# chungongyu/siga

Hardware: AMD Instinct MI355X
Metric: reads/sec overlapped (ASQG bit-exact) (higher is better)
Workload: dtype u64

## Files before the change

siga_amd/csrc/sigax_kernels.hip:

```cpp
#include <hip/hip_runtime.h>

#include <cstdlib>

#include "sigax_kernels.h"

typedef unsigned long long u64;
typedef unsigned int u32;

#ifndef SIGAX_NT
#define SIGAX_NT 7
#endif

struct Cnt4 {
  u64 a, c, g, t;
};

template <bool WIDE> struct PosOf { typedef u32 type; };
template <> struct PosOf<true> { typedef u64 type; };
template <typename P> struct Cnt4P {
  P a, c, g, t;
};

template <bool WIDE> struct Cand;
template <> struct __attribute__((aligned(32))) Cand<false> {
// ... 604 lines not shown
      }
      return true;
    }
    slot = slot + 1 == nslots ? 0 : slot + 1;
  }
}

__device__ __forceinline__ void store_block(sigax_block* dst, u64 c0lo, u64 c0hi, u64 c1lo, u64 c1hi, u64 r0lo, u64 r0hi,
                                            u64 r1lo, u64 r1hi, u32 len, u32 af) {
  ulonglong2* d = reinterpret_cast<ulonglong2*>(dst);
  d[0] = make_ulonglong2(c0lo, c0hi);
  d[1] = make_ulonglong2(c1lo, c1hi);
  d[2] = make_ulonglong2(r0lo, r0hi);
  d[3] = make_ulonglong2(r1lo, r1hi);
  d[4] = make_ulonglong2((u64)len | ((u64)af << 32), 0ull);
}

template <bool WIDE>
__global__ __launch_bounds__(256) void k_build2_a(FmStrand s, u32* gran2, u32* cnt, u64 ng2) {
  const FmRef F = fm_ref(s, 0);
  const u32 lane = threadIdx.x & 63u;
  const u64 wave = ((u64)blockIdx.x * 256 + threadIdx.x) >> 6, nw = (u64)gridDim.x * 4;
  for (u64 g = wave; g < ng2; g += nw) {
    const u64 p = g * 64 + lane;
    u32 c1 = 0, c2 = 0;
    if (p < s.n) {
      c1 = fm_char(F, p);
      if (c1 >= 1 && c1 <= 4) {
        const Cnt4 k = fm_rank<WIDE>(F, p);
        const u64 rk = c1 == 1 ? k.a : c1 == 2 ? k.c : c1 == 3 ? k.g : k.t;
        c2 = fm_char(F, s.C[c1] + rk);
      } else {
        c1 = c1 > 4 ? 0 : c1;
      }
    }
    const u64 y1 = __ballot((c1 & 1u) != 0), z1 = __ballot((c1 & 2u) != 0), w1 = __ballot((c1 & 4u) != 0);
    const u64 y2 = __ballot((c2 & 1u) != 0), z2 = __ballot((c2 & 2u) != 0), w2 = __ballot((c2 & 4u) != 0);
    u32 mine = 0;
    for (u32 b = 1; b <= 4; ++b) {
      const u32 v = (u32)__popcll(__ballot(c1 == b));
      if (lane == b - 1) mine = v;
    }
    for (u32 c = 1; c <= 4; ++c)
      for (u32 x = 1; x <= 4; ++x) {
        const u32 v = (u32)__popcll(__ballot(c1 == c && c2 == x));
        if (lane == 4 + (c - 1) * 4 + (x - 1)) mine = v;
      }
    if (lane < 20) cnt[(u64)lane * ng2 + g] = mine;
    if (lane == 0) {
      u32* q = gran2 + g * SIGAX_GRAN2_WORDS + 20;
      q[0] = (u32)y1; q[1] = (u32)(y1 >> 32); q[2] = (u32)z1; q[3] = (u32)(z1 >> 32); q[4] = (u32)w1; q[5] = (u32)(w1 >> 32);
      q[6] = (u32)y2; q[7] = (u32)(y2 >> 32); q[8] = (u32)z2; q[9] = (u32)(z2 >> 32); q[10] = (u32)w2; q[11] = (u32)(w2 >> 32);
    }
  }
}
__global__ __launch_bounds__(256) void k_build2_b(const u64* offs, u32* gran2, u32 col, u64 ng2, u64* super2) {
  const u64 g = (u64)blockIdx.x * 256 + threadIdx.x;
  if (g >= ng2) return;
  u64 base = 0;
  if (super2) {
    const u32 sh = SIGAX_SUPER_SHIFT - 6;
    const u64 first = (g >> sh) << sh;
    base = offs[first];
    if (g == first) super2[(g >> sh) * 20 + col] = base;
  }
  gran2[g * SIGAX_GRAN2_WORDS + col] = (u32)(offs[g] - base);
}

#ifndef SIGAX_FIND_POLICY
#define SIGAX_FIND_POLICY ""
#endif
struct Gran2 {
  v4u s, pc, p5, p6, p7;
};
__device__ __forceinline__ void find_step2_loads(const void* base, u32 offa, u32 offa_c, u32 offb, u32 offb_c, Gran2& a, Gran2& b) {
  asm volatile(
      "global_load_dwordx4 %0, %10, %14" SIGAX_FIND_POLICY "\n\t"
      "global_load_dwordx4 %5, %12, %14" SIGAX_FIND_POLICY "\n\t"
      "global_load_dwordx4 %1, %11, %14" SIGAX_FIND_POLICY "\n\t"
      "global_load_dwordx4 %2, %10, %14 offset:80" SIGAX_FIND_POLICY "\n\t"
      "global_load_dwordx4 %3, %10, %14 offset:96" SIGAX_FIND_POLICY "\n\t"
      "global_load_dwordx4 %4, %10, %14 offset:112" SIGAX_FIND_POLICY "\n\t"
      "global_load_dwordx4 %6, %13, %14" SIGAX_FIND_POLICY "\n\t"
      "global_load_dwordx4 %7, %12, %14 offset:80" SIGAX_FIND_POLICY "\n\t"
      "global_load_dwordx4 %8, %12, %14 offset:96" SIGAX_FIND_POLICY "\n\t"
      "global_load_dwordx4 %9, %12, %14 offset:112" SIGAX_FIND_POLICY "\n\t"
      "s_waitcnt vmcnt(0)"
      : "=&v"(a.s), "=&v"(a.pc), "=&v"(a.p5), "=&v"(a.p6), "=&v"(a.p7), "=&v"(b.s), "=&v"(b.pc), "=&v"(b.p5), "=&v"(b.p6),
        "=&v"(b.p7)
      : "v"(offa), "v"(offa_c), "v"(offb), "v"(offb_c), "s"(base)
      : "memory");
}
__device__ __forceinline__ void find_step2_loads_masked(const void* base, u32 offa, u32 offa_c, u32 offb, u32 offb_c, u64 two, Gran2& a,
                                                        Gran2& b) {
  u64 saved;
  asm volatile(
      "global_load_dwordx4 %0, %11, %15" SIGAX_FIND_POLICY "\n\t"
      "global_load_dwordx4 %1, %12, %15" SIGAX_FIND_POLICY "\n\t"
      "global_load_dwordx4 %2, %11, %15 offset:80" SIGAX_FIND_POLICY "\n\t"
      "global_load_dwordx4 %3, %11, %15 offset:96" SIGAX_FIND_POLICY "\n\t"
      "global_load_dwordx4 %4, %11, %15 offset:112" SIGAX_FIND_POLICY "\n\t"
      "s_and_saveexec_b64 %10, %16\n\t"
      "global_load_dwordx4 %5, %13, %15" SIGAX_FIND_POLICY "\n\t"
      "global_load_dwordx4 %6, %14, %15" SIGAX_FIND_POLICY "\n\t"
      "global_load_dwordx4 %7, %13, %15 offset:80" SIGAX_FIND_POLICY "\n\t"
      "global_load_dwordx4 %8, %13, %15 offset:96" SIGAX_FIND_POLICY "\n\t"
      "global_load_dwordx4 %9, %13, %15 offset:112" SIGAX_FIND_POLICY "\n\t"
      "s_mov_b64 exec, %10\n\t"
      "s_waitcnt vmcnt(0)"
      : "=&v"(a.s), "=&v"(a.pc), "=&v"(a.p5), "=&v"(a.p6), "=&v"(a.p7), "=&v"(b.s), "=&v"(b.pc), "=&v"(b.p5), "=&v"(b.p6),
        "=&v"(b.p7), "=&s"(saved)
      : "v"(offa), "v"(offa_c), "v"(offb), "v"(offb_c), "s"(base), "s"(two)
      : "memory", "scc");
}
#define COOP_A_U4 512u
#define COOP_B_U4 128u
#define COOP_WAVE_U4 (COOP_A_U4 + COOP_B_U4 + 16u)
__device__ __forceinline__ void find_step2_dma(const uint32_t* gran2, u32 la, u32 lb, u32 c, uint4* stage, u32 lane, Gran2& a, Gran2& b) {
  const u32 j = lane & 7u, pp = lane >> 3;
  const char* base = reinterpret_cast<const char*>(gran2);
  u32* list = reinterpret_cast<u32*>(stage + COOP_A_U4 + COOP_B_U4);
  const bool differ = lb != la;
  const u64 dmask = __ballot(differ);
  const u32 nd = (u32)__popcll(dmask);
  const u32 r = (u32)__popcll(dmask & ((1ull << lane) - 1ull));
  asm volatile("s_waitcnt lgkmcnt(0)" ::: "memory");
  if (differ) list[r] = lb;
#pragma unroll
  for (u32 t = 0; t < 8; ++t) {
    const u32 lA = (u32)__shfl((int)la, (int)(8u * t + j), 64);
    const u32 p = pp ^ (t & 1u);
    const char* sa = base + (u64)lA * 128u + p * 16u;
    __builtin_amdgcn_global_load_lds((const __attribute__((address_space(1))) void*)sa,
                                     (__attribute__((address_space(3))) void*)(u32)(size_t)(stage + t * 64u), 16, 0, 0);
  }
  const u32 tt = lane >> 3, x = tt & 1u;
  auto ld = [](const uint4* q) { const uint4 v = *q; v4u w; w.x = v.x; w.y = v.y; w.z = v.z; w.w = v.w; return w; };
  bool gotA = false;
  const u32 npass = (nd + 15u) >> 4;
  for (u32 ps = 0; ps < npass || !gotA; ++ps) {
    if (ps < npass) {
      asm volatile("s_waitcnt lgkmcnt(0)" ::: "memory");
      __builtin_amdgcn_fence(__ATOMIC_ACQ_REL, "wavefront");
      __builtin_amdgcn_wave_barrier();
#pragma unroll
      for (u32 t = 0; t < 2; ++t) {
        const u32 rk = 16u * ps + 8u * t + j;
        if (rk < nd) {
          const u32 lB = list[rk];
          const u32 p = pp ^ (t & 1u);
          const char* sb = base + (u64)lB * 128u + p * 16u;
          __builtin_amdgcn_global_load_lds((const __attribute__((address_space(1))) void*)sb,
                                           (__attribute__((address_space(3))) void*)(u32)(size_t)(stage + COOP_A_U4 + t * 64u), 16, 0, 0);
        }
      }
    }
    asm volatile("s_waitcnt vmcnt(0)" ::: "memory");
    __builtin_amdgcn_fence(__ATOMIC_ACQUIRE, "wavefront");
    __builtin_amdgcn_wave_barrier();
    if (!gotA) {
      const uint4* qa = stage + tt * 64u + j;
      a.s = ld(qa + ((0u ^ x) * 8u)); a.pc = ld(qa + ((c ^ x) * 8u)); a.p5 = ld(qa + ((5u ^ x) * 8u)); a.p6 = ld(qa + ((6u ^ x) * 8u)); a.p7 = ld(qa + ((7u ^ x) * 8u));
      gotA = true;
    }
    if (differ && (r >> 4) == ps) {
      const u32 q = r & 15u, tb = q >> 3, xb = tb & 1u;
      const uint4* qb = stage + COOP_A_U4 + tb * 64u + (q & 7u);
      b.s = ld(qb + ((0u ^ xb) * 8u)); b.pc = ld(qb + ((c ^ xb) * 8u)); b.p5 = ld(qb + ((5u ^ xb) * 8u)); b.p6 = ld(qb + ((6u ^ xb) * 8u)); b.p7 = ld(qb + ((7u ^ xb) * 8u));
    }
  }
  asm volatile("s_waitcnt lgkmcnt(0)" ::: "memory");
  if (!differ) b = a;
}

struct Rank2 {
  u32 a, c, g, t;
  u32 pa, pc, pg, pt;
};
__device__ __forceinline__ Rank2 rank2_from(const Gran2& q, u32 r, u32 c) {
  const u32 m0 = r >= 32 ? 0xFFFFFFFFu : ((1u << r) - 1u);
  const u32 m1 = r > 32 ? ((1u << (r - 32)) - 1u) : 0u;
  const bool cb0 = ((c - 1u) & 1u) != 0, cb1 = ((c - 1u) & 2u) != 0;
  Rank2 o;
  o.a = q.s.x; o.c = q.s.y; o.g = q.s.z; o.t = q.s.w;
  o.pa = q.pc.x; o.pc = q.pc.y; o.pg = q.pc.z; o.pt = q.pc.w;
  auto word = [&](u32 y, u32 z, u32 w, u32 y2, u32 z2, u32 w2, u32 m) {
    const u32 A = y & ~z, C = z & ~y, G = y & z, T = w;
    o.a += __popc(A & m); o.c += __popc(C & m); o.g += __popc(G & m); o.t += __popc(T & m);
    const u32 E = (cb1 ? (cb0 ? T : G) : (cb0 ? C : A)) & m;
    o.pa += __popc(y2 & ~z2 & E); o.pc += __popc(z2 & ~y2 & E); o.pg += __popc(y2 & z2 & E); o.pt += __popc(w2 & E);
  };
  word(q.p5.x, q.p5.z, q.p6.x, q.p6.z, q.p7.x, q.p7.z, m0);
  word(q.p5.y, q.p5.w, q.p6.y, q.p6.w, q.p7.y, q.p7.w, m1);
  return o;
}
template <bool WIDE>
struct Find2TablesT {
  typedef typename PosOf<WIDE>::type P;
  P Cc[2][4][4];
  P Cd[2][4];
};
typedef Find2TablesT<false> Find2Tables;
template <bool WIDE>
__device__ __forceinline__ void find2_tables_load(Find2TablesT<WIDE>& t, const FmStrand& fwd, const FmStrand& rev) {
  typedef typename PosOf<WIDE>::type P;
  if (threadIdx.x < 8) {
    const u32 which = threadIdx.x >> 2, c = (threadIdx.x & 3u) + 1u;
    const FmStrand& st = which ? rev : fwd;
    const FmRef F = fm_ref(st, which);
    const u64 pos = st.C[c];
    const Cnt4 k = fm_rank<WIDE>(F, pos);
    t.Cc[which][c - 1][0] = (P)k.a; t.Cc[which][c - 1][1] = (P)k.c; t.Cc[which][c - 1][2] = (P)k.g; t.Cc[which][c - 1][3] = (P)k.t;
    t.Cd[which][c - 1] = (P)(pos - (k.a + k.c + k.g + k.t));
  }
}

template <int NT>
struct FindStageT {
  static constexpr bool direct = false;
  uint4 row_[NT][4];
  u64 tag_[NT];
  __device__ __forceinline__ uint4* row(u32 t) { return row_[t]; }
  __device__ __forceinline__ u64& tag(u32 t) { return tag_[t]; }
};
typedef FindStageT<256> FindStage;
typedef FindStageT<128> FindStageC;
struct FindStageNone {
  static constexpr bool direct = true;
  __device__ __forceinline__ uint4* row(u32) { return nullptr; }
  __device__ __forceinline__ u64& tag(u32) { return dummy; }
  u64 dummy;
};

template <class SG>
__device__ __forceinline__ void find_flush(SG& sg, bool want, u32 tid) {
  if constexpr (SG::direct) return;
  const u32 lane = tid & 63u, q0 = tid & ~3u, piece = tid & 3u;
  __builtin_amdgcn_wave_barrier();
  u64 bal = __ballot(want);
  u32 qm = (u32)(bal >> (lane & 60u)) & 0xFu;
  while (__ballot(qm != 0) != 0) {
    if (qm != 0) {
      const u32 src = q0 + (u32)__builtin_ctz(qm);
      const u64 tag = sg.tag(src);
      if (piece <= (u32)(tag & 3u)) {
        const uint4 v = sg.row(src)[piece];
#if (SIGAX_NT & 2)
        {
          typedef u32 nt4 __attribute__((ext_vector_type(4)));
          nt4 w;
          w.x = v.x; w.y = v.y; w.z = v.z; w.w = v.w;
          __builtin_nontemporal_store(w, reinterpret_cast<nt4*>((tag & ~(u64)3) + piece * 16u));
        }
#else
        *reinterpret_cast<uint4*>((tag & ~(u64)3) + piece * 16u) = v;
#endif
      }
      qm &= qm - 1u;
    }
  }
  __builtin_amdgcn_wave_barrier();
}

__device__ __forceinline__ u32 rd_rank(const unsigned char* rd, u32 i) { return ((u32)rd[i >> 1] >> ((i & 1u) * 4u)) & 15u; }

template <bool WIDE, bool STAGED, bool TWO, bool COOP = false, int NT = 256, class SG = FindStage>
__device__ __forceinline__ void find_body(const FindArgs& A, FmTables& tb, SG& sg, const Find2TablesT<WIDE>& t2,
                                          const unsigned char* rd, u64 rd_base, uint4* coop_stage = nullptr, u32 tile = blockIdx.x) {
  const u32 tid = threadIdx.x;
  const u32 wv = __builtin_amdgcn_readfirstlane(tid >> 6);
  const u32 o = A.chain_base + (wv & (A.chains_per_wg - 1u));
  const u32 wslot = (wv / A.chains_per_wg) * 64u + (tid & 63u);
  const u32 slot = A.read_begin + tile * ((u32)NT / A.chains_per_wg) + wslot;
  const bool inr = slot < A.read_end;
  const u32 read = (A.perm != nullptr && inr) ? A.perm[slot] : slot;
  typedef typename PosOf<WIDE>::type P;
  u32 nocc = 0;
  u32 nsec = 0;
  u32 nb = 0, flagbits = 0;
  bool live = inr && ((A.chain_mask >> o) & 1u);
  u64 b0 = 0;
  u32 L = 0;
  if (live) {
    b0 = A.offs[read];
    L = (u32)(A.offs[read + 1] - b0);
    live = L > 0;
  }
  const bool pf = o < 2;
  const FmRef F = fm_ref(A.fwd, 0), R = fm_ref(A.rev, 1);
  const FmRef PI = fm_pick(pf, F, R);
  const FmRef OI = fm_pick(pf, R, F);
  const u64* CP = tb.C[PI.which];
  const u64* CO = tb.C[OI.which];
  const void* PI2 = pf ? (const void*)A.fwd.gran2 : (const void*)A.rev.gran2;
  const u64* PS2 = pf ? A.fwd.super2 : A.rev.super2;
  const bool comp = (o & 1u) != 0;
  const bool fromStart = (o == 1 || o == 2);
  const u32 af = o == 0 ? SIGAX_AF_CHAIN0 : o == 1 ? SIGAX_AF_CHAIN1 : o == 2 ? SIGAX_AF_CHAIN2 : SIGAX_AF_CHAIN3;
  const unsigned char* sq = A.seqs + b0;
  const u32 rdo = A.perm != nullptr ? wslot * A.stage_stride : (u32)(b0 - rd_base);
  const u64 b0w = ((u64)__builtin_amdgcn_readfirstlane((u32)(b0 >> 32)) << 32) | __builtin_amdgcn_readfirstlane((u32)b0);
  const unsigned char* sq0 = A.seqs + b0w;
  const u32 sqd = (u32)(b0 - b0w);
  auto slot_addr = [&](u32 i) -> u64 {
    return reinterpret_cast<u64>(A.arena) + (((u64)read * 4 + o) * A.cap + i) * sizeof(Cand<WIDE>);
  };

  P lo0 = 0, sz = 0, lo1 = 0;
  u32 s = 1;
  bool started = false;
  if (STAGED && A.deep_k != 0u) {
    const u32 K = A.deep_k;
    const bool can = live && L >= K;
    if (__ballot(can) != 0) {
      u64 k0 = 0, k1 = 0;
      bool acgt = can;
      for (u32 i = 0; i < K; ++i) {
        u32 r = 1u;
        if (can) {
          const u32 at = rdo + (fromStart ? i : L - 1u - i);
          r = COOP ? rd_rank(rd, at) : base_rank(rd[at]);
        }
        if (comp) r = comp_rank(r);
        acgt = acgt && r != 0u;
        const u64 c = (u64)((r - 1u) & 3u);
        if (i < 32u) k0 |= c << (2u * i);
        else k1 |= c << (2u * (i - 32u));
      }
      if (acgt) {
        k1 |= (u64)(0x8000u | K) << 48;
        P a0 = 0, a1 = 0, az = 0;
        if (deep_lookup<WIDE>(pf ? A.fwd.deep : A.rev.deep, pf ? A.fwd.deep_slots : A.rev.deep_slots, k0, k1, a0, a1, az)) {
          lo0 = a0; lo1 = a1; sz = az; s = K;
          started = true;
        }
      }
    }
  }
  if (STAGED && live && !started && A.start_ok && L >= (u32)SIGAX_START_K) {
    const void* ST = pf ? A.fwd.start : A.rev.start;
    u32 code = 0;
    bool acgt = true;
#pragma unroll
    for (u32 i = 0; i < (u32)SIGAX_START_K; ++i) {
      const u32 at = rdo + (fromStart ? i : L - 1u - i);
      u32 r = COOP ? rd_rank(rd, at) : base_rank(rd[at]);
      if (comp) r = comp_rank(r);
      acgt = acgt && r != 0u;
      code = (code << 2) | ((r - 1u) & 3u);
    }
    if (acgt) {
      if (WIDE) {
        const ulonglong2* q = reinterpret_cast<const ulonglong2*>(ST) + 2ull * code;
        const ulonglong2 a = q[0], b = q[1];
        lo0 = (P)a.x; lo1 = (P)a.y; sz = (P)b.x; s = (u32)b.y;
      } else {
        const uint4 e = reinterpret_cast<const uint4*>(ST)[code];
        lo0 = (P)e.x; lo1 = (P)e.y; sz = (P)e.z; s = e.w;
      }
      started = true;
    }
  }
  nsec += (u32)__popcll(__ballot(started));
  if (live && !started) {
    u32 r = (STAGED && COOP) ? rd_rank(rd, rdo + (fromStart ? 0 : L - 1)) : base_rank(STAGED ? rd[rdo + (fromStart ? 0 : L - 1)] : sq[fromStart ? 0 : L - 1]);
    if (comp) r = comp_rank(r);
    lo0 = (P)CP[r]; sz = (P)tb.T[PI.which][r]; lo1 = (P)CO[r];
  }
  bool full = !live;
  auto emit = [&](P c0lo, P d, P c1lo, P r0lo, P szv, u32 len) -> bool {
    bool fl = false;
    if constexpr (SG::direct) {
      if (nb < A.cap - 1 && !full) {
        cand_store(reinterpret_cast<Cand<WIDE>*>(slot_addr(nb)), c0lo, d, c1lo, r0lo, c1lo, szv, len, af);
      } else {
        flagbits |= 1u;
        full = true;
      }
      ++nb;
      return false;
    }
    if (nb < A.cap - 1 && !full) {
      if (WIDE) {
        cand_store(reinterpret_cast<Cand<WIDE>*>(sg.row(tid)), c0lo, d, c1lo, r0lo, c1lo, szv, len, af);
        sg.tag(tid) = slot_addr(nb) | 3u;
        fl = true;
      } else {
        cand_store(reinterpret_cast<Cand<WIDE>*>(sg.row(tid) + (nb & 1u) * 2), c0lo, d, c1lo, r0lo, c1lo, szv, len, af);
        if (nb & 1u) {
          sg.tag(tid) = slot_addr(nb - 1) | 3u;
          fl = true;
        }
      }
    } else {
      flagbits |= 1u;
      full = true;
    }
    ++nb;
    return fl;
  };
  for (;;) {
    const bool on = live && sz != 0 && s < L;
    if (__ballot(on) == 0) break;
    if (TWO) {
      u32 c = 0, e = 0;
      const bool want2 = on && s + 1 < L;
      if (want2) {
        if (COOP) {
          c = rd_rank(rd, rdo + (fromStart ? s : L - 1 - s));
          e = rd_rank(rd, rdo + (fromStart ? s + 1 : L - 2 - s));
        } else {
          c = base_rank(rd[rdo + (fromStart ? s : L - 1 - s)]);
          e = base_rank(rd[rdo + (fromStart ? s + 1 : L - 2 - s)]);
        }
        if (comp) { c = comp_rank(c); e = comp_rank(e); }
      }
      const bool ok2 = want2 && c != 0 && e != 0;
      if (__ballot(on && !ok2) == 0) {
        bool fl1 = false, fl2 = false, two_lines = false;
        P lo1n = 0, lo0n = 0, szn = 0, ldn = 0, dd2 = 0, nlo1 = 0, nlo0 = 0, nsz = 0;
        Gran2 ga, gb;
        P pl = 0, pu = 0;
        if (on) {
          const P nn = (P)PI.n;
          pl = lo0 > nn ? nn : lo0;
          const P up = (P)(lo0 + sz);
          pu = (up > nn || up < lo0) ? nn : up;
          two_lines = (pl >> 6) != (pu >> 6);
        }
        const u64 two_mask = COOP ? 0ull : __ballot(two_lines);
        if (COOP) {
          find_step2_dma(reinterpret_cast<const uint32_t*>(PI2), (u32)(pl >> 6), (u32)(pu >> 6), on ? c : 1u,
                         coop_stage + wv * COOP_WAVE_U4, tid & 63u, ga, gb);
        }
        if (on) {
          if (!COOP) {
            const u32 oa = (u32)(pl >> 6) * 128u, ob = (u32)(pu >> 6) * 128u;
            if (A.mask_upper) {
              find_step2_loads_masked(PI2, oa, oa + 16u * c, ob, ob + 16u * c, two_mask, ga, gb);
              if (!two_lines) gb = ga;
            } else {
              find_step2_loads(PI2, oa, oa + 16u * c, ob, ob + 16u * c, ga, gb);
            }
          }
          const Rank2 lr = rank2_from(ga, (u32)pl & 63u, c), ur = rank2_from(gb, (u32)pu & 63u, c);
          P la = lr.a, lcn = lr.c, lg = lr.g, lt = lr.t, ua = ur.a, ucn = ur.c, ug = ur.g, ut = ur.t;
          P lpa = lr.pa, lpc = lr.pc, lpg = lr.pg, lpt = lr.pt, upa = ur.pa, upc = ur.pc, upg = ur.pg, upt = ur.pt;
          if (WIDE) {
            const u64* sl = PS2 + ((u64)pl >> SIGAX_SUPER_SHIFT) * 20;
            const u64* su = PS2 + ((u64)pu >> SIGAX_SUPER_SHIFT) * 20;
            const u32 pb = 4u + (c - 1u) * 4u;
            la += (P)sl[0]; lcn += (P)sl[1]; lg += (P)sl[2]; lt += (P)sl[3];
            ua += (P)su[0]; ucn += (P)su[1]; ug += (P)su[2]; ut += (P)su[3];
            lpa += (P)sl[pb]; lpc += (P)sl[pb + 1]; lpg += (P)sl[pb + 2]; lpt += (P)sl[pb + 3];
            upa += (P)su[pb]; upc += (P)su[pb + 1]; upg += (P)su[pb + 2]; upt += (P)su[pb + 3];
          }
          const P da = ua - la, dc = ucn - lcn, dg = ug - lg, dt = ut - lt;
          const P dd = sz - (da + dc + dg + dt);
          const P ld = lo0 - (la + lcn + lg + lt);
          if (s >= A.minov && dd > 0) fl1 = emit(ld, dd, lo1, lo0, sz, s);
          const P acc1 = sel5<P>(c, (P)0, dd, dd + da, dd + da + dc, dd + da + dc + dg);
          const P lc = sel5<P>(c, ld, la, lcn, lg, lt);
          const P dcc = sel5<P>(c, dd, da, dc, dg, dt);
          lo1n = lo1 + acc1;
          lo0n = (P)CP[c] + lc;
          szn = dcc;
          const P d2a = upa - lpa, d2c = upc - lpc, d2g = upg - lpg, d2t = upt - lpt;
          const P l2d = lc - (lpa + lpc + lpg + lpt);
          dd2 = dcc - (d2a + d2c + d2g + d2t);
          ldn = t2.Cd[PI.which][c - 1] + l2d;
          const P acc2 = sel5<P>(e, (P)0, dd2, dd2 + d2a, dd2 + d2a + d2c, dd2 + d2a + d2c + d2g);
          const P l2e = sel5<P>(e, (P)0, lpa, lpc, lpg, lpt);
          const P d2e = sel5<P>(e, (P)0, d2a, d2c, d2g, d2t);
          nlo1 = lo1n + acc2;
          nlo0 = (P)CP[e] + t2.Cc[PI.which][c - 1][e - 1] + l2e;
          nsz = d2e;
        }
        nsec += 2u * (u32)(__popcll(__ballot(on)) + __popcll(__ballot(two_lines)));
        find_flush(sg, fl1, tid);
        if (on) {
          if (s + 1 >= A.minov && dd2 > 0) fl2 = emit(ldn, dd2, lo1n, lo0n, szn, s + 1);
          lo1 = nlo1; lo0 = nlo0; sz = nsz;
          s += szn != 0 ? 2u : 1u;
        }
        find_flush(sg, fl2, tid);
        continue;
      }
    }
    bool flush = false, two_gran = false;
    if (on) {
      const u64 pl = (u64)lo0 > PI.n ? PI.n : (u64)lo0;
      const u64 pu0 = (u64)(P)(lo0 + sz);
      const u64 pu = pu0 > PI.n ? PI.n : pu0;
      Gran gl, gu;
      u32 ch;
      two_gran = (pl >> 7) != (pu >> 7);
      if (STAGED) {
        ch = COOP ? rd_rank(rd, rdo + (fromStart ? s : L - 1 - s)) : (u32)rd[rdo + (fromStart ? s : L - 1 - s)];
        if (WIDE) find_step_loads8(PI.g + (pl >> 7) * 4, PI.g + (pu >> 7) * 4, gl, gu);
        else find_step_loads8_s(PI.g, (u32)(pl >> 7) * 64u, (u32)(pu >> 7) * 64u, gl, gu);
      } else if (WIDE) {
        find_step_loads(PI.g + (pl >> 7) * 4, PI.g + (pu >> 7) * 4, sq + (fromStart ? s : L - 1 - s), gl, gu, ch);
      } else {
        find_step_loads_s(PI.g, (u32)(pl >> 7) * 64u, (u32)(pu >> 7) * 64u, sq0, sqd + (fromStart ? s : L - 1 - s), gl, gu, ch);
      }
      const Cnt4P<P> l = fm_rank4p_from<WIDE>(PI, pl, gl);
      const Cnt4P<P> u = fm_rank4p_from<WIDE>(PI, pu, gu);
      u32 r = (STAGED && COOP) ? ch : base_rank(ch & 0xFFu);
      if (comp) r = comp_rank(r);
      P da = u.a - l.a, dc = u.c - l.c, dg = u.g - l.g, dt = u.t - l.t;
      P dd = sz - (da + dc + dg + dt);
      const P ld = lo0 - (l.a + l.c + l.g + l.t);
      if (s >= A.minov && dd > 0) flush = emit(ld, dd, lo1, lo0, sz, s);
      const P p1 = dd, p2 = dd + da, p3 = p2 + dc, p4 = p3 + dg;
      const P acc = sel5<P>(r, (P)0, p1, p2, p3, p4);
      const P lc = sel5<P>(r, ld, l.a, l.c, l.g, l.t);
      const P dcur = sel5<P>(r, dd, da, dc, dg, dt);
      lo1 += acc;
      lo0 = (P)CP[r] + lc;
      sz = dcur;
      ++s;
    }
    nsec += (u32)(__popcll(__ballot(on)) + __popcll(__ballot(two_gran)));
    find_flush(sg, flush, tid);
  }
  {
    const bool tail = !WIDE && live && !full && (nb & 1u);
    if (!SG::direct && tail) sg.tag(tid) = slot_addr(nb - 1) | 1u;
    find_flush(sg, tail, tid);
  }
  bool contain = false;
  u32 tail_sec = 0;
  nocc = live ? 2u * (s - 1u) : 0u;
  if (live && sz != 0 && s >= L) {
    auto clampn = [](u64 p, u64 n) { return p > n ? n : p; };
    const u64 pl = clampn((u64)lo0, PI.n), pu = clampn((u64)(P)(lo0 + sz), PI.n);
    const u64 ql = clampn((u64)lo1, OI.n), qu = clampn((u64)(P)(lo1 + sz), OI.n);
    Gran ga, gb;
    u32 ignored;
    tail_sec = ((pl >> 7) != (pu >> 7) ? 2u : 1u) + ((ql >> 7) != (qu >> 7) ? 2u : 1u);
    find_step_loads(PI.g + (pl >> 7) * 4, PI.g + (pu >> 7) * 4, sq, ga, gb, ignored);
    const Cnt4P<P> l = fm_rank4p_from<WIDE>(PI, pl, ga);
    const Cnt4P<P> u = fm_rank4p_from<WIDE>(PI, pu, gb);
    find_step_loads(OI.g + (ql >> 7) * 4, OI.g + (qu >> 7) * 4, sq, ga, gb, ignored);
    const Cnt4P<P> lp = fm_rank4p_from<WIDE>(OI, ql, ga);
    const Cnt4P<P> up = fm_rank4p_from<WIDE>(OI, qu, gb);
    nocc += 4;
    bool dna = (u.a - l.a) | (u.c - l.c) | (u.g - l.g) | (u.t - l.t) | (up.a - lp.a) | (up.c - lp.c) | (up.g - lp.g) |
               (up.t - lp.t);
    if (dna) {
      flagbits |= SIGAX_CC_SUBSTRING;
    } else {
      P ld = lo0 - (l.a + l.c + l.g + l.t);
      P lpd = lo1 - (lp.a + lp.c + lp.g + lp.t);
      if constexpr (SG::direct) {
        cand_store(reinterpret_cast<Cand<WIDE>*>(slot_addr(A.cap - 1)), ld, sz, lpd, lo0, lo1, sz, L, af);
      } else {
        cand_store(reinterpret_cast<Cand<WIDE>*>(sg.row(tid)), ld, sz, lpd, lo0, lo1, sz, L, af);
        sg.tag(tid) = slot_addr(A.cap - 1) | (WIDE ? 3u : 1u);
      }
      flagbits |= SIGAX_CC_CONTAIN;
      contain = true;
    }
  }
  find_flush(sg, contain, tid);
  if (inr) {
    const u32 nbw = (flagbits & 1u) ? 0u : nb;
    u32 word = (nbw & SIGAX_CC_COUNT_MASK) | (flagbits & (SIGAX_CC_SUBSTRING | SIGAX_CC_CONTAIN));
    A.chain_cnt[(u64)read * 4 + o] = word;
  }
  u64 tot_occ = wave_sum((u64)nocc);
  u64 tot_blk = wave_sum((u64)nb + ((flagbits & SIGAX_CC_CONTAIN) ? 1u : 0u));
  u64 tot_err = wave_sum((u64)(flagbits & 1u));
  u64 tot_sec = (u64)nsec + wave_sum((u64)tail_sec);
  u32 mx = nb;
  for (int off = 32; off > 0; off >>= 1) mx = max(mx, (u32)__shfl_xor((int)mx, off, 64));
  if ((threadIdx.x & 63) == 0) {
    if (mx > A.max_seen) atomicMax(&A.dstat[DS_MAX_CHAIN], (u64)mx);
    if (tot_sec) atomicAdd(&A.dstat[DS_SEC_FIND], tot_sec);
    if (tot_occ) atomicAdd(&A.dstat[DS_OCC_FIND], tot_occ);
    if (tot_blk) atomicAdd(&A.dstat[DS_CAND_BLOCKS], tot_blk);
    if (tot_err) atomicAdd(&A.dstat[DS_FIND_OVERFLOW], tot_err);
  }
}

extern __shared__ __attribute__((aligned(16))) unsigned char find_dyn_lds[];
template <int NT = 256>
__device__ __forceinline__ bool find_stage_reads(const FindArgs& A, u64* rd_base) {
  const u32 per = (u32)NT / A.chains_per_wg;
  const u32 r0 = A.read_begin + blockIdx.x * per;
  const u32 r1 = r0 + per < A.read_end ? r0 + per : A.read_end;
  const u64 lo = A.offs[r0], hi = A.offs[r1];
  const u64 alo = (reinterpret_cast<u64>(A.seqs) + lo) & ~3ull;
  const u64 nbytes = reinterpret_cast<u64>(A.seqs) + hi - alo;
  *rd_base = alo - reinterpret_cast<u64>(A.seqs);
  if (nbytes + 4 > (u64)A.stage_bytes) return false;
  const u32* src = reinterpret_cast<const u32*>(alo);
  u32* dst = reinterpret_cast<u32*>(find_dyn_lds);
  const u32 nw = (u32)((nbytes + 3) >> 2);
  for (u32 w = threadIdx.x; w < nw; w += (u32)NT) dst[w] = src[w];
  return true;
}

template <int NT>
__device__ __forceinline__ bool find_stage_reads_perm(const FindArgs& A, u32 tile) {
  const u32 per = (u32)NT / A.chains_per_wg;
  if ((u64)per * A.stage_stride > (u64)A.stage_bytes) return false;
  const u32 r0 = A.read_begin + tile * per;
  const u32 j = threadIdx.x;
  if (j < per && r0 + j < A.read_end) {
    const u32 r = A.perm[r0 + j];
    const u64 b = A.offs[r];
    const u32 len = (u32)(A.offs[r + 1] - b);
    const unsigned char* src = A.seqs + b;
    unsigned char* d = find_dyn_lds + j * A.stage_stride;
    const u32 nw = len >> 2;
    for (u32 k = 0; k < nw; ++k) {
      u32 w;
      __builtin_memcpy(&w, src + 4u * k, 4);
      reinterpret_cast<u32*>(d)[k] = w;
    }
    for (u32 i = nw << 2; i < len; ++i) d[i] = src[i];
  }
  return true;
}

template <int NT>
__device__ __forceinline__ bool find_stage_reads_packed(const FindArgs& A, u64* rd_base, u32 tile) {
  const u32 per = (u32)NT / A.chains_per_wg;
  const u32 r0 = A.read_begin + tile * per;
  const u32 r1 = r0 + per < A.read_end ? r0 + per : A.read_end;
  const u64 lo = A.offs[r0], hi = A.offs[r1];
  const u64 alo = (reinterpret_cast<u64>(A.seqs) + lo) & ~3ull;
  const u64 nbytes = reinterpret_cast<u64>(A.seqs) + hi - alo;
  *rd_base = alo - reinterpret_cast<u64>(A.seqs);
  if ((nbytes + 3) / 2 + 4 > (u64)A.stage_bytes) return false;
  const u32* src = reinterpret_cast<const u32*>(alo);
  unsigned short* dst = reinterpret_cast<unsigned short*>(find_dyn_lds);
  const u32 nw = (u32)((nbytes + 3) >> 2);
  for (u32 w = threadIdx.x; w < nw; w += (u32)NT) {
    const u32 v = src[w];
    dst[w] = (unsigned short)(base_rank(v & 0xFFu) | (base_rank((v >> 8) & 0xFFu) << 4) | (base_rank((v >> 16) & 0xFFu) << 8) |
                              (base_rank(v >> 24) << 12));
  }
  return true;
}

template <int NT>
__device__ __forceinline__ bool find_stage_reads_packed_perm(const FindArgs& A, u32 tile) {
  const u32 per = (u32)NT / A.chains_per_wg;
  if ((u64)per * A.stage_stride / 2u > (u64)A.stage_bytes) return false;
  const u32 r0 = A.read_begin + tile * per;
  const u32 j = threadIdx.x;
  if (j < per && r0 + j < A.read_end) {
    const u32 r = A.perm[r0 + j];
    const u64 b = A.offs[r];
    const u32 len = (u32)(A.offs[r + 1] - b);
    const unsigned char* src = A.seqs + b;
    unsigned char* d = find_dyn_lds + j * (A.stage_stride / 2u);
    const u32 nw = len >> 2;
    for (u32 k = 0; k < nw; ++k) {
      u32 v;
      __builtin_memcpy(&v, src + 4u * k, 4);
      reinterpret_cast<unsigned short*>(d)[k] = (unsigned short)(base_rank(v & 0xFFu) | (base_rank((v >> 8) & 0xFFu) << 4) |
                                                                 (base_rank((v >> 16) & 0xFFu) << 8) | (base_rank(v >> 24) << 12));
    }
    for (u32 i = nw << 2; i < len; ++i) {
      const u32 rk = base_rank(src[i]);
      const u32 old = (i & 1u) ? d[i >> 1] : 0u;
      d[i >> 1] = (unsigned char)((i & 1u) ? ((old & 0x0Fu) | (rk << 4)) : rk);
    }
  }
  return true;
}

__global__ __launch_bounds__(256) __attribute__((amdgpu_waves_per_eu(8, 8))) void k_find_n(FindArgs A) {
  __shared__ FmTables tb;
  __shared__ FindStage sg;
  __shared__ Find2Tables t2;
  u64 rd_base = 0;
  const bool staged = A.perm != nullptr ? find_stage_reads_perm<256>(A, blockIdx.x) : find_stage_reads(A, &rd_base);
  fm_tables_load(tb, A.fwd, A.rev);
  if (staged) find_body<false, true, false>(A, tb, sg, t2, find_dyn_lds, rd_base);
  else find_body<false, false, false>(A, tb, sg, t2, find_dyn_lds, rd_base);
}
__global__ __launch_bounds__(256) void k_find_n2(FindArgs A) {
  __shared__ FmTables tb;
  __shared__ FindStage sg;
  __shared__ Find2Tables t2;
  u64 rd_base = 0;
  const bool staged = A.perm != nullptr ? find_stage_reads_perm<256>(A, blockIdx.x) : find_stage_reads(A, &rd_base);
  find2_tables_load(t2, A.fwd, A.rev);
  fm_tables_load(tb, A.fwd, A.rev);
#ifdef SIGAX_FIND_PRIO
  __builtin_amdgcn_s_setprio(SIGAX_FIND_PRIO);
#endif
  if (staged) find_body<false, true, true>(A, tb, sg, t2, find_dyn_lds, rd_base);
  else find_body<false, false, false>(A, tb, sg, t2, find_dyn_lds, rd_base);
}
__global__ __launch_bounds__(128) void k_find_c2(FindArgs A) {
  __shared__ FmTables tb;
  __shared__ Find2Tables t2;
  __shared__ __attribute__((aligned(16))) uint4 stage[2 * COOP_WAVE_U4];
  find2_tables_load(t2, A.fwd, A.rev);
  fm_tables_load(tb, A.fwd, A.rev);
  const u32 ntiles = (A.read_end - A.read_begin + 63u) / 64u;
  for (u32 tile = blockIdx.x; tile < ntiles; tile += gridDim.x) {
    u64 rd_base = 0;
    const bool staged = A.perm != nullptr ? find_stage_reads_packed_perm<128>(A, tile) : find_stage_reads_packed<128>(A, &rd_base, tile);
    __syncthreads();
    FindStageNone sg;
    if (staged) find_body<false, true, true, true, 128, FindStageNone>(A, tb, sg, t2, find_dyn_lds, rd_base, stage, tile);
    else find_body<false, false, false, false, 128, FindStageNone>(A, tb, sg, t2, find_dyn_lds, rd_base, stage, tile);
    __syncthreads();
  }
}
__global__ __launch_bounds__(128) void k_find_c2w(FindArgs A) {
  __shared__ FmTables tb;
  __shared__ Find2TablesT<true> t2;
  __shared__ __attribute__((aligned(16))) uint4 stage[2 * COOP_WAVE_U4];
  find2_tables_load<true>(t2, A.fwd, A.rev);
  fm_tables_load(tb, A.fwd, A.rev);
  const u32 ntiles = (A.read_end - A.read_begin + 63u) / 64u;
  for (u32 tile = blockIdx.x; tile < ntiles; tile += gridDim.x) {
    u64 rd_base = 0;
    const bool staged = A.perm != nullptr ? find_stage_reads_packed_perm<128>(A, tile) : find_stage_reads_packed<128>(A, &rd_base, tile);
    __syncthreads();
    FindStageNone sg;
    if (staged) find_body<true, true, true, true, 128, FindStageNone>(A, tb, sg, t2, find_dyn_lds, rd_base, stage, tile);
    else find_body<true, false, false, false, 128, FindStageNone>(A, tb, sg, t2, find_dyn_lds, rd_base, stage, tile);
    __syncthreads();
  }
}
__global__ __launch_bounds__(256) void k_find_w(FindArgs A) {
  __shared__ FmTables tb;
  __shared__ FindStage sg;
  __shared__ Find2TablesT<true> t2;
  u64 rd_base = 0;
  const bool staged = A.perm != nullptr ? find_stage_reads_perm<256>(A, blockIdx.x) : find_stage_reads(A, &rd_base);
  fm_tables_load(tb, A.fwd, A.rev);
  if (staged) find_body<true, true, false>(A, tb, sg, t2, find_dyn_lds, rd_base);
  else find_body<true, false, false>(A, tb, sg, t2, find_dyn_lds, rd_base);
}

#define FX_COUNTDOWN 0x80000000u
struct Ent {
  u64 c0lo, c0hi, c1lo, c1hi;
  u32 src, len;
  u32 pad0, pad1;
};

__device__ __forceinline__ bool iv_valid(u64 lo, u64 hi) { return hi != ~0ull && hi >= lo; }
__device__ __forceinline__ bool intersecting(u64 s1, u64 e1, u64 s2, u64 e2) { return !(s1 > e2 || s2 > e1); }

template <bool WIDE>
struct Fx {
  const FxArgs& A;
  const FmTables& tb;
  FmRef F, R;
  Ent* pool;
  u32 top;
  bool overflow;
  bool xerror;
  u64 nocc;
  u32 read, nout;
  const Cand<WIDE>* slots;

  __device__ Fx(const FxArgs& a, const FmTables& t, Ent* p)
      : A(a), tb(t), F(fm_ref(a.fwd, 0)), R(fm_ref(a.rev, 1)), pool(p), top(0), overflow(false), xerror(false), nocc(0),
        read(0), nout(0), slots(nullptr) {}

  __device__ u32 af_of(u32 src) const {
    u32 ch = src / A.cap;
    return ch == 0 ? SIGAX_AF_CHAIN0 : ch == 1 ? SIGAX_AF_CHAIN1 : ch == 2 ? SIGAX_AF_CHAIN2 : SIGAX_AF_CHAIN3;
  }
  __device__ FmRef ext_index(u32 src) const { return fm_pick((src / A.cap) < 2, R, F); }

  __device__ bool need(u32 upto) {
    if (upto + nout > A.pool_cap) { overflow = true; return false; }
    return true;
  }

  __device__ void load_ent(Ent& e, u32 src) const {
    const Cand<WIDE> b = cand_load<WIDE>(slots + src);
    e.c0lo = b.c0lo; e.c0hi = (u64)b.c0lo + b.d - 1; e.c1lo = b.c1lo; e.c1hi = (u64)b.c1lo + b.d - 1;
    e.src = src; e.len = b.len; e.pad0 = e.pad1 = 0;
  }

  __device__ void emit(const Ent& e) {
    if (top + nout + 1 > A.pool_cap) { overflow = true; return; }
    pool[A.pool_cap - 1 - nout] = e;
    ++nout;
  }
  __device__ void flush(u64& fin_cur, u64& fin_end) {
    if (fin_cur + nout > fin_end) {
      u64 grab = nout > 64 ? nout : 64;
      fin_cur = atomicAdd(&A.dstat[DS_FIN_TOP], grab);
      fin_end = fin_cur + grab;
    }
    A.item_base[2ull * read] = fin_cur;
    for (u32 i = 0; i < nout; ++i) {
      u64 slot = fin_cur + i;
      if (slot >= A.fin_cap) break;
      const Ent& e = pool[A.pool_cap - 1 - i];
      const Cand<WIDE> b = cand_load<WIDE>(slots + e.src);
      store_block(A.fin + slot, e.c0lo, e.c0hi, e.c1lo, e.c1hi, b.r0lo, (u64)b.r0lo + b.sz - 1, b.r1lo, (u64)b.r1lo + b.sz - 1, b.len, b.af);
    }
    fin_cur += nout;
  }

  __device__ void updateR(Ent& e, u32 r, const FmRef& ix) {
    u64 l[5], u[5];
    fm_rank5<WIDE>(ix, e.c1lo, l);
    fm_rank5<WIDE>(ix, e.c1hi + 1, u);
    u64 acc = 0, lr = 0, ur = 0;
    for (u32 b = 0; b < 5; ++b) {
      if (b < r) acc += u[b] - l[b];
      if (b == r) { lr = l[b]; ur = u[b]; }
    }
    u64 pb = tb.C[ix.which][r];
    e.c0lo += acc;
    e.c0hi = e.c0lo + (ur - lr) - 1;
    e.c1lo = pb + lr;
    e.c1hi = pb + ur - 1;
  }
  __device__ void updateL(Ent& e, u32 r, const FmRef& ix) {
    u64 l[5], u[5];
    fm_rank5<WIDE>(ix, e.c0lo, l);
    fm_rank5<WIDE>(ix, e.c0hi + 1, u);
    u64 acc = 0, lr = 0, ur = 0;
    for (u32 b = 0; b < 5; ++b) {
      if (b < r) acc += u[b] - l[b];
      if (b == r) { lr = l[b]; ur = u[b]; }
    }
    u64 pb = tb.C[ix.which][r];
    e.c1lo += acc;
    e.c1hi = e.c1lo + (ur - lr) - 1;
    e.c0lo = pb + lr;
    e.c0hi = pb + ur - 1;
  }
  __device__ void ext(const Ent& e, u64 x[5]) {
    FmRef ix = ext_index(e.src);
    u64 l[5], u[5];
    fm_rank5<WIDE>(ix, e.c1lo, l);
    fm_rank5<WIDE>(ix, e.c1hi + 1, u);
    for (int k = 0; k < 5; ++k) x[k] = u[k] - l[k];
    if (af_of(e.src) & 4u) {
      u64 t = x[1]; x[1] = x[4]; x[4] = t;
      t = x[2]; x[2] = x[3]; x[3] = t;
    }
  }

  __device__ void sort_left(u32 base, u32 n) {
    for (u32 i = 1; i < n; ++i) {
      Ent k = pool[base + i];
      u32 j = i;
      while (j > 0 && k.c0lo < pool[base + j - 1].c0lo) { pool[base + j] = pool[base + j - 1]; --j; }
      pool[base + j] = k;
    }
  }
  __device__ void sort_len_desc(u32 base, u32 n) {
    for (u32 i = 1; i < n; ++i) {
      Ent k = pool[base + i];
      u32 j = i;
      while (j > 0 && k.len > pool[base + j - 1].len) { pool[base + j] = pool[base + j - 1]; --j; }
      pool[base + j] = k;
    }
  }

  __device__ u32 resolve(const Ent& x, const Ent& y, u32 rb, u32 rcap, const FmRef& Pfm, const FmRef& Ofm) {
    const Ent* higher = &x;
    const Ent* lower = &y;
    if (higher->len < lower->len) { const Ent* t = higher; higher = lower; lower = t; }
    u32 k = 0;
    pool[rb + k++] = *higher;
    if (higher->len == lower->len) return k;
    if (!(lower->c0lo < higher->c0lo || lower->c0hi > higher->c0hi)) return k;
    const Cand<WIDE> lb = cand_load<WIDE>(slots + lower->src);
    u64* used = reinterpret_cast<u64*>(pool + rb + rcap);
    u32 nused = 0;
    for (u64 j = lower->c1lo; j <= lower->c1hi; ++j) {
      Ent ti;
      ti.c0lo = lb.r0lo; ti.c0hi = (u64)lb.r0lo + lb.sz - 1; ti.c1lo = lb.r1lo; ti.c1hi = (u64)lb.r1lo + lb.sz - 1;
      ti.src = lower->src; ti.len = lower->len; ti.pad0 = ti.pad1 = 0;
      u64 tlo = j, thi = j;
      bool done = false;
      u32 guard = 0;
      while (!done) {
        u32 c = fm_char(Ofm, tlo);
        if (c == 0) {
          updateL(ti, 0, Pfm);
          nocc += 2;
          done = true;
        }
        u64 l[5], u[5];
        fm_rank5<WIDE>(Ofm, tlo, l);
        fm_rank5<WIDE>(Ofm, thi + 1, u);
        u64 lr = 0, ur = 0;
        for (u32 b = 0; b < 5; ++b)
          if (b == c) { lr = l[b]; ur = u[b]; }
        u64 pb = tb.C[Ofm.which][c];
        tlo = pb + lr;
        thi = pb + ur - 1;
        updateR(ti, c, Ofm);
        nocc += 4;
        if (++guard > (1u << 20)) { overflow = true; return k; }
      }
      u64 forward;
      if (ti.c0lo == ti.c0hi) {
        forward = ti.c0lo;
      } else {
        u64 key = ti.c0lo, idx = key;
        u32 f = 0;
        for (; f < nused; ++f)
          if (used[2 * f] == key) break;
        if (f < nused) idx = used[2 * f + 1];
        forward = idx;
        if (f == nused) { used[2 * f] = key; ++nused; }
        used[2 * f + 1] = idx + 1;
      }
      if (!intersecting(forward, forward, higher->c0lo, higher->c0hi)) {
        if (k >= rcap) { overflow = true; return k; }
        Ent sp = *lower;
        sp.c0lo = forward; sp.c0hi = forward; sp.c1lo = j; sp.c1hi = j;
        pool[rb + k++] = sp;
      }
    }
    return k;
  }

  __device__ u32 filter(u32 base, u32 n, const FmRef& Pfm, const FmRef& Ofm) {
    if (n == 0) return 0;
    sort_left(base, n);
    u32 prev = 0, curr = 1;
    u32 guard = 0;
    while (curr < n) {
      Ent a = pool[base + prev];
      Ent b = pool[base + curr];
      if (intersecting(a.c0lo, a.c0hi, b.c0lo, b.c0hi)) {
        const Ent& lower = (a.len < b.len) ? a : b;
        u64 w = lower.c1hi - lower.c1lo + 1;
        if (w > A.pool_cap) { overflow = true; return n; }
        u32 rcap = (u32)w + 1;
        u32 rb = base + n + rcap;
        if (!need(rb + rcap + (rcap * 16 + (u32)sizeof(Ent) - 1) / (u32)sizeof(Ent))) return n;
        u32 k = resolve(a, b, rb, rcap, Pfm, Ofm);
        if (overflow) return n;
        for (u32 i = 1; i < k; ++i) {
          Ent key = pool[rb + i];
          u32 j = i;
          while (j > 0 && key.c0lo < pool[rb + j - 1].c0lo) { pool[rb + j] = pool[rb + j - 1]; --j; }
          pool[rb + j] = key;
        }
        for (u32 i = prev; i + 2 < n; ++i) pool[base + i] = pool[base + i + 2];
        n -= 2;
        int i = (int)n - 1, j = (int)k - 1;
        u32 dst = n + k;
        while (j >= 0) {
          if (i >= 0 && pool[rb + j].c0lo < pool[base + i].c0lo) pool[base + --dst] = pool[base + i--];
          else pool[base + --dst] = pool[rb + j--];
        }
        n += k;
        prev = 0;
        if (++guard > (1u << 16)) { overflow = true; return n; }
      } else {
        ++prev;
      }
      curr = prev + 1;
    }
    return n;
  }

  __device__ u32 updateR_list(u32 off, u32 cnt, u32 c) {
    u32 w = 0;
    for (u32 i = 0; i < cnt; ++i) {
      Ent e = pool[off + i];
      u32 b = (af_of(e.src) & 4u) ? comp_rank(c) : c;
      updateR(e, b, ext_index(e.src));
      if (iv_valid(e.c0lo, e.c0hi) && iv_valid(e.c1lo, e.c1hi)) pool[off + w++] = e;
    }
    return w;
  }

  __device__ bool extract(u32 base, u32 n) {
    sort_len_desc(base, n);
    top = base + n;
    const u32 GMAX = A.pool_cap / 12 > 32 ? A.pool_cap / 12 : 32;
    u32 dents = (GMAX * 2 * (u32)sizeof(uint2) + (u32)sizeof(Ent) - 1) / (u32)sizeof(Ent);
    if (!need(top + dents)) return true;
    uint2* D = reinterpret_cast<uint2*>(pool + top);
    uint2* I = D + GMAX;
    top += dents;
    u32 ng = 1;
    D[0] = make_uint2(base, n);
    u32 guard = 0;
    while (ng > 0) {
      u32 ni = 0;
      u32 p = 0;
      while (p != ng) {
        u32 off = D[p].x, cnt = D[p].y;
        bool eraseGroup = true;
        if (cnt & FX_COUNTDOWN) {
          Ent& g = pool[off];
          if (g.c1hi == 0 || ng == 1 || (ng == 2 && p == 0 && ni == 0)) {
            nocc += 2 * (g.c1hi + 1);
            Ent br = g;
            br.c0hi = br.c0lo;
            br.c1hi = br.c1lo;
            emit(br);
          } else {
            g.c1hi -= 1;
            nocc += 2;
            eraseGroup = false;
          }
        } else if (cnt > 0) {
          u64 exts[5] = {0, 0, 0, 0, 0};
          u32 topLen = pool[off].len;
          u32 ntop = 0;
          for (; ntop < cnt && pool[off + ntop].len == topLen; ++ntop) {
            u64 x[5];
            ext(pool[off + ntop], x);
            nocc += 2;
            for (int k = 0; k < 5; ++k) exts[k] += x[k];
          }
          if (exts[0] > 0) {
            for (u32 j = 0; j < ntop; ++j) {
              u64 x[5];
              ext(pool[off + j], x);
              if (x[0] == 0) { xerror = true; return false; }
              Ent br = pool[off + j];
              updateR(br, 0, ext_index(br.src));
              emit(br);
            }
          } else {
            for (u32 j = ntop; j < cnt; ++j) {
              u64 x[5];
              ext(pool[off + j], x);
              nocc += 2;
              for (int k = 0; k < 5; ++k) exts[k] += x[k];
            }
            int nz = 0, first = -1;
            for (int k = 0; k < 5; ++k)
// ... 2174 lines not shown
```

Baseline: 152.1 million.

## Stage reads as pre-ranked nibbles and simplify base indexing in find

```diff
diff --git a/siga_amd/csrc/sigax_kernels.hip b/siga_amd/csrc/sigax_kernels.hip
--- a/siga_amd/csrc/sigax_kernels.hip
+++ b/siga_amd/csrc/sigax_kernels.hip
@@ -930,9 +930,10 @@
   const u64 b0w = ((u64)__builtin_amdgcn_readfirstlane((u32)(b0 >> 32)) << 32) | __builtin_amdgcn_readfirstlane((u32)b0);
   const unsigned char* sq0 = A.seqs + b0w;
   const u32 sqd = (u32)(b0 - b0w);
-  auto slot_addr = [&](u32 i) -> u64 {
-    return reinterpret_cast<u64>(A.arena) + (((u64)read * 4 + o) * A.cap + i) * sizeof(Cand<WIDE>);
-  };
+  const u64 slot0 = reinterpret_cast<u64>(A.arena) + ((u64)read * 4 + o) * A.cap * sizeof(Cand<WIDE>);
+  auto slot_addr = [&](u32 i) -> u64 { return slot0 + i * (u32)sizeof(Cand<WIDE>); };
+  const u32 rb = rdo + (fromStart ? 0u : L);
+  const u32 rx = fromStart ? 0u : ~0u;
 
   P lo0 = 0, sz = 0, lo1 = 0;
   u32 s = 1;
@@ -942,20 +943,17 @@
     const bool can = live && L >= K;
     if (__ballot(can) != 0) {
       u64 k0 = 0, k1 = 0;
-      bool acgt = can;
+      const u32 codes = comp ? 0x01230u : 0x32100u;
+      const u32 rbk = can ? rb : K + 1u;
+      u32 rmin = 4u;
       for (u32 i = 0; i < K; ++i) {
-        u32 r = 1u;
-        if (can) {
-          const u32 at = rdo + (fromStart ? i : L - 1u - i);
-          r = COOP ? rd_rank(rd, at) : base_rank(rd[at]);
-        }
-        if (comp) r = comp_rank(r);
-        acgt = acgt && r != 0u;
-        const u64 c = (u64)((r - 1u) & 3u);
+        const u32 r = rd_rank(rd, rbk + (i ^ rx));
+        rmin = r < rmin ? r : rmin;
+        const u64 c = (u64)((codes >> (4u * r)) & 3u);
         if (i < 32u) k0 |= c << (2u * i);
         else k1 |= c << (2u * (i - 32u));
       }
-      if (acgt) {
+      if (can && rmin != 0u) {
         k1 |= (u64)(0x8000u | K) << 48;
         P a0 = 0, a1 = 0, az = 0;
         if (deep_lookup<WIDE>(pf ? A.fwd.deep : A.rev.deep, pf ? A.fwd.deep_slots : A.rev.deep_slots, k0, k1, a0, a1, az)) {
@@ -971,8 +969,7 @@
     bool acgt = true;
 #pragma unroll
     for (u32 i = 0; i < (u32)SIGAX_START_K; ++i) {
-      const u32 at = rdo + (fromStart ? i : L - 1u - i);
-      u32 r = COOP ? rd_rank(rd, at) : base_rank(rd[at]);
+      u32 r = rd_rank(rd, rb + (i ^ rx));
       if (comp) r = comp_rank(r);
       acgt = acgt && r != 0u;
       code = (code << 2) | ((r - 1u) & 3u);
@@ -991,7 +988,7 @@
   }
   nsec += (u32)__popcll(__ballot(started));
   if (live && !started) {
-    u32 r = (STAGED && COOP) ? rd_rank(rd, rdo + (fromStart ? 0 : L - 1)) : base_rank(STAGED ? rd[rdo + (fromStart ? 0 : L - 1)] : sq[fromStart ? 0 : L - 1]);
+    u32 r = STAGED ? rd_rank(rd, rb + rx) : base_rank(sq[fromStart ? 0 : L - 1]);
     if (comp) r = comp_rank(r);
     lo0 = (P)CP[r]; sz = (P)tb.T[PI.which][r]; lo1 = (P)CO[r];
   }
@@ -1037,13 +1034,21 @@
         if (COOP) {
           c = rd_rank(rd, rdo + (fromStart ? s : L - 1 - s));
           e = rd_rank(rd, rdo + (fromStart ? s + 1 : L - 2 - s));
+          if (comp) { c = comp_rank(c); e = comp_rank(e); }
         } else {
-          c = base_rank(rd[rdo + (fromStart ? s : L - 1 - s)]);
-          e = base_rank(rd[rdo + (fromStart ? s + 1 : L - 2 - s)]);
-        }
-        if (comp) { c = comp_rank(c); e = comp_rank(e); }
+          const u32 i0 = rb + (s ^ rx) - (fromStart ? 0u : 1u);
+          unsigned short w;
+          __builtin_memcpy(&w, rd + (i0 >> 1), 2);
+          const u32 sh = (i0 & 1u) * 4u;
+          c = ((u32)w >> (sh + (fromStart ? 0u : 4u))) & 15u;
+          e = ((u32)w >> (sh + (fromStart ? 4u : 0u))) & 15u;
+        }
       }
       const bool ok2 = want2 && c != 0 && e != 0;
+      if constexpr (!COOP) {
+        c = (c ^ (comp ? ~0u : 0u)) + (comp ? 6u : 0u);
+        e = (e ^ (comp ? ~0u : 0u)) + (comp ? 6u : 0u);
+      }
       if (__ballot(on && !ok2) == 0) {
         bool fl1 = false, fl2 = false, two_lines = false;
         P lo1n = 0, lo0n = 0, szn = 0, ldn = 0, dd2 = 0, nlo1 = 0, nlo0 = 0, nsz = 0;
@@ -1051,9 +1056,9 @@
         P pl = 0, pu = 0;
         if (on) {
           const P nn = (P)PI.n;
-          pl = lo0 > nn ? nn : lo0;
           const P up = (P)(lo0 + sz);
-          pu = (up > nn || up < lo0) ? nn : up;
+          pl = lo0 < nn ? lo0 : nn;
+          pu = up < nn ? up : nn;
           two_lines = (pl >> 6) != (pu >> 6);
         }
         const u64 two_mask = COOP ? 0ull : __ballot(two_lines);
@@ -1124,7 +1129,7 @@
       u32 ch;
       two_gran = (pl >> 7) != (pu >> 7);
       if (STAGED) {
-        ch = COOP ? rd_rank(rd, rdo + (fromStart ? s : L - 1 - s)) : (u32)rd[rdo + (fromStart ? s : L - 1 - s)];
+        ch = rd_rank(rd, rb + (s ^ rx));
         if (WIDE) find_step_loads8(PI.g + (pl >> 7) * 4, PI.g + (pu >> 7) * 4, gl, gu);
         else find_step_loads8_s(PI.g, (u32)(pl >> 7) * 64u, (u32)(pu >> 7) * 64u, gl, gu);
       } else if (WIDE) {
@@ -1134,7 +1139,7 @@
       }
       const Cnt4P<P> l = fm_rank4p_from<WIDE>(PI, pl, gl);
       const Cnt4P<P> u = fm_rank4p_from<WIDE>(PI, pu, gu);
-      u32 r = (STAGED && COOP) ? ch : base_rank(ch & 0xFFu);
+      u32 r = STAGED ? ch : base_rank(ch & 0xFFu);
       if (comp) r = comp_rank(r);
       P da = u.a - l.a, dc = u.c - l.c, dg = u.g - l.g, dt = u.t - l.t;
       P dd = sz - (da + dc + dg + dt);
@@ -1213,47 +1218,10 @@
 }
 
 extern __shared__ __attribute__((aligned(16))) unsigned char find_dyn_lds[];
-template <int NT = 256>
-__device__ __forceinline__ bool find_stage_reads(const FindArgs& A, u64* rd_base) {
-  const u32 per = (u32)NT / A.chains_per_wg;
-  const u32 r0 = A.read_begin + blockIdx.x * per;
-  const u32 r1 = r0 + per < A.read_end ? r0 + per : A.read_end;
-  const u64 lo = A.offs[r0], hi = A.offs[r1];
-  const u64 alo = (reinterpret_cast<u64>(A.seqs) + lo) & ~3ull;
-  const u64 nbytes = reinterpret_cast<u64>(A.seqs) + hi - alo;
-  *rd_base = alo - reinterpret_cast<u64>(A.seqs);
-  if (nbytes + 4 > (u64)A.stage_bytes) return false;
-  const u32* src = reinterpret_cast<const u32*>(alo);
-  u32* dst = reinterpret_cast<u32*>(find_dyn_lds);
-  const u32 nw = (u32)((nbytes + 3) >> 2);
-  for (u32 w = threadIdx.x; w < nw; w += (u32)NT) dst[w] = src[w];
-  return true;
-}
-
-template <int NT>
-__device__ __forceinline__ bool find_stage_reads_perm(const FindArgs& A, u32 tile) {
-  const u32 per = (u32)NT / A.chains_per_wg;
-  if ((u64)per * A.stage_stride > (u64)A.stage_bytes) return false;
-  const u32 r0 = A.read_begin + tile * per;
-  const u32 j = threadIdx.x;
-  if (j < per && r0 + j < A.read_end) {
-    const u32 r = A.perm[r0 + j];
-    const u64 b = A.offs[r];
-    const u32 len = (u32)(A.offs[r + 1] - b);
-    const unsigned char* src = A.seqs + b;
-    unsigned char* d = find_dyn_lds + j * A.stage_stride;
-    const u32 nw = len >> 2;
-    for (u32 k = 0; k < nw; ++k) {
-      u32 w;
-      __builtin_memcpy(&w, src + 4u * k, 4);
-      reinterpret_cast<u32*>(d)[k] = w;
-    }
-    for (u32 i = nw << 2; i < len; ++i) d[i] = src[i];
-  }
-  return true;
-}
-
-template <int NT>
+__device__ __forceinline__ u32 pack_ranks4(u32 v) {
+  return base_rank(v & 0xFFu) | (base_rank((v >> 8) & 0xFFu) << 4) | (base_rank((v >> 16) & 0xFFu) << 8) | (base_rank(v >> 24) << 12);
+}
+template <int NT, bool BYTES = false>
 __device__ __forceinline__ bool find_stage_reads_packed(const FindArgs& A, u64* rd_base, u32 tile) {
   const u32 per = (u32)NT / A.chains_per_wg;
   const u32 r0 = A.read_begin + tile * per;
@@ -1262,22 +1230,18 @@
   const u64 alo = (reinterpret_cast<u64>(A.seqs) + lo) & ~3ull;
   const u64 nbytes = reinterpret_cast<u64>(A.seqs) + hi - alo;
   *rd_base = alo - reinterpret_cast<u64>(A.seqs);
-  if ((nbytes + 3) / 2 + 4 > (u64)A.stage_bytes) return false;
+  if ((BYTES ? nbytes : (nbytes + 3) / 2) + 4 > (u64)A.stage_bytes) return false;
   const u32* src = reinterpret_cast<const u32*>(alo);
   unsigned short* dst = reinterpret_cast<unsigned short*>(find_dyn_lds);
   const u32 nw = (u32)((nbytes + 3) >> 2);
-  for (u32 w = threadIdx.x; w < nw; w += (u32)NT) {
-    const u32 v = src[w];
-    dst[w] = (unsigned short)(base_rank(v & 0xFFu) | (base_rank((v >> 8) & 0xFFu) << 4) | (base_rank((v >> 16) & 0xFFu) << 8) |
-                              (base_rank(v >> 24) << 12));
-  }
+  for (u32 w = threadIdx.x; w < nw; w += (u32)NT) dst[w] = (unsigned short)pack_ranks4(src[w]);
   return true;
 }
 
-template <int NT>
+template <int NT, bool BYTES = false>
 __device__ __forceinline__ bool find_stage_reads_packed_perm(const FindArgs& A, u32 tile) {
   const u32 per = (u32)NT / A.chains_per_wg;
-  if ((u64)per * A.stage_stride / 2u > (u64)A.stage_bytes) return false;
+  if ((u64)per * A.stage_stride / (BYTES ? 1u : 2u) > (u64)A.stage_bytes) return false;
   const u32 r0 = A.read_begin + tile * per;
   const u32 j = threadIdx.x;
   if (j < per && r0 + j < A.read_end) {
@@ -1290,8 +1254,7 @@
     for (u32 k = 0; k < nw; ++k) {
       u32 v;
       __builtin_memcpy(&v, src + 4u * k, 4);
-      reinterpret_cast<unsigned short*>(d)[k] = (unsigned short)(base_rank(v & 0xFFu) | (base_rank((v >> 8) & 0xFFu) << 4) |
-                                                                 (base_rank((v >> 16) & 0xFFu) << 8) | (base_rank(v >> 24) << 12));
+      reinterpret_cast<unsigned short*>(d)[k] = (unsigned short)pack_ranks4(v);
     }
     for (u32 i = nw << 2; i < len; ++i) {
       const u32 rk = base_rank(src[i]);
@@ -1300,6 +1263,9 @@
     }
   }
   return true;
+}
+__device__ __forceinline__ bool find_stage_reads(const FindArgs& A, u64* rd_base) {
+  return A.perm != nullptr ? find_stage_reads_packed_perm<256, true>(A, blockIdx.x) : find_stage_reads_packed<256, true>(A, rd_base, blockIdx.x);
 }
 
 __global__ __launch_bounds__(256) __attribute__((amdgpu_waves_per_eu(8, 8))) void k_find_n(FindArgs A) {
@@ -1307,7 +1273,7 @@
   __shared__ FindStage sg;
   __shared__ Find2Tables t2;
   u64 rd_base = 0;
-  const bool staged = A.perm != nullptr ? find_stage_reads_perm<256>(A, blockIdx.x) : find_stage_reads(A, &rd_base);
+  const bool staged = find_stage_reads(A, &rd_base);
   fm_tables_load(tb, A.fwd, A.rev);
   if (staged) find_body<false, true, false>(A, tb, sg, t2, find_dyn_lds, rd_base);
   else find_body<false, false, false>(A, tb, sg, t2, find_dyn_lds, rd_base);
@@ -1317,7 +1283,7 @@
   __shared__ FindStage sg;
   __shared__ Find2Tables t2;
   u64 rd_base = 0;
-  const bool staged = A.perm != nullptr ? find_stage_reads_perm<256>(A, blockIdx.x) : find_stage_reads(A, &rd_base);
+  const bool staged = find_stage_reads(A, &rd_base);
   find2_tables_load(t2, A.fwd, A.rev);
   fm_tables_load(tb, A.fwd, A.rev);
 #ifdef SIGAX_FIND_PRIO
@@ -1365,7 +1331,7 @@
   __shared__ FindStage sg;
   __shared__ Find2TablesT<true> t2;
   u64 rd_base = 0;
-  const bool staged = A.perm != nullptr ? find_stage_reads_perm<256>(A, blockIdx.x) : find_stage_reads(A, &rd_base);
+  const bool staged = find_stage_reads(A, &rd_base);
   fm_tables_load(tb, A.fwd, A.rev);
   if (staged) find_body<true, true, false>(A, tb, sg, t2, find_dyn_lds, rd_base);
   else find_body<true, false, false>(A, tb, sg, t2, find_dyn_lds, rd_base);
```

Measured after the change: 152.1 million. About the same (-0.0%).
